# facebookresearch/PointContrast

Hardware: AMD Instinct MI355X
Metric: scene-pairs/sec, ScanNet 2.5cm Res16UNet34C PointInfoNCE (higher is better)
Workload: dtype f32; 1 GPU; BASELINE configs[1]: Res16UNet34C, nce loss, voxel 0.025 m, 4 pairs/GPU, 87380+87371 active voxels per forward pair on rank 0, npos 4096, T 0.4, SGD(lr 0.1, mom 0.8, wd 1e-4); global_batch=4, parallelism=dp1, engine=native, pair_execution=one two-segment pass (BatchNorm statistics per cloud)

## Files before the change

pointcontrast_amd/csrc/spconv_plan.h:

```cpp
#pragma once
#include <algorithm>
#include <cmath>
#include <cstdlib>

#include "internal.h"
#include "spconv_args.h"

namespace pcmi {

constexpr int kStreamKDefaultMinTiles = 256;

struct ConvEnv {
  int64_t sk_min_tiles, conv16_min_rows, conv32r_min_rows;
  bool x3_on;
};
static ConvEnv conv_env() {
  ConvEnv env;
  const char* e = getenv("PCMI_SPCONV_STREAMK");
  env.sk_min_tiles = e ? (int64_t)atoll(e) : (int64_t)kStreamKDefaultMinTiles;
  e = getenv("PCMI_CONV16");
  env.conv16_min_rows = e ? atoll(e) : 512;
  e = getenv("PCMI_CONV16_X3");
  env.x3_on = !e || atoi(e) != 0;
  e = getenv("PCMI_CONV32R");
  env.conv32r_min_rows = e ? (int64_t)atoll(e) : (int64_t)8192;
  return env;
}

static int sk_workgroups_max() { return 4 * num_cu() / 8 * 8; }
static bool sk_rows_eligible(const ConvEnv& env, int64_t rows, int K) {
  const int64_t mt = env.sk_min_tiles;
  return K > 1 && mt > 0 && rows >= 4096  && ceil_div(rows, 128) >= mt;
}
static size_t sk_partial_bytes(const ConvEnv& env, int64_t rows, int N, int K) {
  return sk_rows_eligible(env, rows, K) ? (size_t)sk_workgroups_max() * 2 * 128 * N * sizeof(float) : 0;
}

static bool conv16_enabled(const ConvEnv& env, int64_t n_rows, int64_t x_bytes) {
  const int64_t min_rows = env.conv16_min_rows;
  return min_rows > 0 && n_rows >= min_rows && x_bytes <= 0x7FFFFF00ll;
}

static bool conv16_x3(const ConvEnv& env, int NT, int C, int N) { return env.x3_on && NT >= 2 && NT <= 4 && C >= 64 && N >= 64; }

struct ConvPlan {
  int kernel;
  int RW, NT, ksplit;
  size_t split_bytes, sk_bytes, pack_offset, pack_bytes;
  size_t ws_bytes;
};
constexpr int kMaxKSplit = 27;

static ConvPlan plan_conv(const ConvEnv& env, int64_t rows, int64_t x_bytes, int C, int N, int K, int form) {
  ConvPlan p = {};
  const bool pair = form == PCMI_CONV_FORM_PAIRS, table = form == PCMI_CONV_FORM_TABLE || form == PCMI_CONV_FORM_TABLE_UNITS;
  p.ksplit = 1;
  if (conv32r_eligible(env.conv32r_min_rows, rows, x_bytes, C, N, K, table)) {
    p.kernel = PCMI_CONV_KERNEL_32R;
    return p;
  }
  const bool wide = C >= 64;
  const int nt_all = N / 32;
  p.NT = nt_all % 4 == 0 ? 4 : (nt_all % 3 == 0 ? 3 : (nt_all % 2 == 0 ? 2 : 1));
  p.RW = rows >= 96 ? 4 : (rows >= 48 ? 2 : 1);
  if (p.RW == 1 && p.NT > 2) p.NT = (nt_all % 2 == 0) ? 2 : 1;
  const int64_t min16 = env.conv16_min_rows;
  if (rows < 2048)
    p.NT = (wide && !pair && K > 1 && N >= 64 && nt_all % 2 == 0 && env.x3_on && min16 > 0 && rows >= min16 && p.RW == 4) ? 2 : 1;
  else if (rows < 8192 && p.NT > 2)
    p.NT = (nt_all % 2 == 0) ? 2 : 1;
  if (pair) {
    p.kernel = PCMI_CONV_KERNEL_PAIR;
    return p;
  }
  if (K > 1 && rows > 0) {
    const int64_t wgs = ceil_div(rows, 32 * p.RW) * (nt_all / p.NT);
    const int64_t target = (25 * (int64_t)num_cu()) / 10;
    if (wgs < target) p.ksplit = (int)std::min<int64_t>(std::min<int64_t>(K, kMaxKSplit), ceil_div(target, wgs));
    if (wide && p.RW == 4 && wgs < target && rows < 16384 && conv16_x3(env, p.NT, C, N) && min16 > 0 && rows >= min16) {
      const double slots = (double)x3_workgroups(p.NT, 3), nch = (double)(C / 32);
      const double traffic = (double)rows * N * 8.0 / 3.0e6 / 2.0;
      auto cost = [&](int ks) {
        const double w = (double)wgs * ks;
        const double rounds = std::ceil(w / slots);
        const double thin = std::max(1.0, 2.0 * num_cu() / std::min(w, slots));
        return rounds * ((double)ceil_div((int64_t)K, (int64_t)ks) * nch + 3.0) * thin + traffic * ks;
      };
      int best = p.ksplit;
      const int kmax = (int)std::min<int64_t>(K, kMaxKSplit);
      for (int ks = 1; ks <= kmax; ++ks)
        if (cost(ks) < cost(best) - 1e-9) best = ks;
      if (cost(best) < 0.9 * cost(p.ksplit)) p.ksplit = best;
    }
  }
  const bool c16 = p.RW == 4 && conv16_enabled(env, rows, x_bytes), x3 = conv16_x3(env, p.NT, C, N);
  if (form == PCMI_CONV_FORM_TABLE_UNITS && c16 && p.ksplit == 1 && sk_rows_eligible(env, rows, K) && C >= 64 && N >= 64) {
    p.kernel = x3 ? PCMI_CONV_KERNEL_UNITS_X3 : PCMI_CONV_KERNEL_UNITS_16;
    p.sk_bytes = sk_partial_bytes(env, rows, N, K);
    p.pack_offset = p.sk_bytes;
    p.pack_bytes = x3 ? x3_pack_bytes(K, C, N) : 0;
    p.ws_bytes = p.pack_offset + p.pack_bytes;
    return p;
  }
  p.split_bytes = p.ksplit > 1 ? (size_t)p.ksplit * rows * N * sizeof(float) : 0;
  p.ws_bytes = p.split_bytes;
  if (c16 && x3 && form != PCMI_CONV_FORM_NONE) {
    p.kernel = PCMI_CONV_KERNEL_TABLE_X3;
    p.pack_offset = align_up(p.split_bytes, 256);
    p.pack_bytes = x3_pack_bytes(K, C, N);
    p.ws_bytes = p.pack_offset + p.pack_bytes;
  } else if (c16) {
    p.kernel = PCMI_CONV_KERNEL_TABLE_16;
  } else if (p.RW == 4 && p.NT <= 2 && C % 64 == 0) {
    p.kernel = PCMI_CONV_KERNEL_DEEP;
  } else {
    p.kernel = PCMI_CONV_KERNEL_PLAIN;
  }
  return p;
}

}
```

pointcontrast_amd/csrc/spconv_x3.hip:

```cpp
#include <algorithm>
#include <cstdio>
#include <cstdlib>

#include "common.h"
#include "internal.h"
#include "spconv_args.h"
#include "x3_split.h"

namespace pcmi {

__host__ __device__ constexpr int x3_piece(int n, int kk) { return (n >> 4) * 64 + kk * 16 + (n & 15); }

__host__ __device__ constexpr int x3_channel(int kk, int e) { return 4 * kk + (e & 3) + 16 * (e >> 2); }

template <int TERMS>
__global__ __launch_bounds__(256) void x3_pack_kernel(const float* __restrict__ w, int64_t w_kstride, int64_t w_sc, int64_t w_sn,
                                                      int K, int C, int N, int NS, u32x4* __restrict__ out) {
  const int nch = C / kKC, nns = N / NS;
  const int64_t total = (int64_t)K * nch * nns * NS * 4;
  const int64_t idx = (int64_t)blockIdx.x * 256 + threadIdx.x;
  if (idx >= total) return;
  const int kk = (int)(idx & 3);
  int64_t r = idx >> 2;
  const int nl = (int)(r % NS);
  r /= NS;
  const int ns = (int)(r % nns);
  r /= nns;
  const int cc = (int)(r % nch);
  const int wk = (int)(r / nch);
  const float* wb = w + (int64_t)wk * w_kstride + (int64_t)(ns * NS + nl) * w_sn;
  v4f x0, x1;
#pragma unroll
  for (int e = 0; e < 4; ++e) {
    x0[e] = wb[(int64_t)(cc * kKC + x3_channel(kk, e)) * w_sc];
    x1[e] = wb[(int64_t)(cc * kKC + x3_channel(kk, e + 4)) * w_sc];
  }
  u32x4 h, m, l;
  split_terms<TERMS>(x0, x1, h, m, l);
  u32x4* blk = out + (((int64_t)wk * nch + cc) * nns + ns) * (TERMS * NS * 4);
  const int piece = x3_piece(nl, kk);
  blk[0 * NS * 4 + piece] = h;
  if constexpr (TERMS == 3) {
    blk[1 * NS * 4 + piece] = m;
    blk[2 * NS * 4 + piece] = l;
  }
}

__global__ __launch_bounds__(256) void x3_pack_many_kernel(const X3PackJob* __restrict__ jobs, int n_jobs, int64_t total,
                                                           int64_t item0) {
  const int64_t idx = item0 + (int64_t)blockIdx.x * 256 + threadIdx.x;
  if (idx >= total) return;
  int lo = 0, hi = n_jobs - 1;
  while (lo < hi) {
    const int mid = (lo + hi + 1) >> 1;
    if (jobs[mid].first_item <= idx) lo = mid; else hi = mid - 1;
  }
  const X3PackJob jb = jobs[lo];
  const int64_t loc = idx - jb.first_item;
  const int nch = jb.C / kKC, nns = jb.N / jb.NS;
  const int kk = (int)(loc & 3);
  int64_t r = loc >> 2;
  const int nl = (int)(r % jb.NS);
  r /= jb.NS;
  const int ns = (int)(r % nns);
  r /= nns;
  const int cc = (int)(r % nch);
  const int wk = (int)(r / nch);
  const float* wb = jb.w + (int64_t)wk * jb.w_kstride + (int64_t)(ns * jb.NS + nl) * jb.w_sn;
  v4f x0, x1;
#pragma unroll
  for (int e = 0; e < 4; ++e) {
    x0[e] = wb[(int64_t)(cc * kKC + x3_channel(kk, e)) * jb.w_sc];
    x1[e] = wb[(int64_t)(cc * kKC + x3_channel(kk, e + 4)) * jb.w_sc];
  }
  const int piece = x3_piece(nl, kk);
  if (jb.terms == 1) {
    u32x4 h;
    split1(x0, x1, h);
    reinterpret_cast<u32x4*>(jb.out)[(((int64_t)wk * nch + cc) * nns + ns) * (jb.NS * 4) + piece] = h;
    return;
  }
  u32x4 h, m, l;
  split3(x0, x1, h, m, l);
  u32x4* blk = reinterpret_cast<u32x4*>(jb.out) + (((int64_t)wk * nch + cc) * nns + ns) * (3 * jb.NS * 4);
  blk[0 * jb.NS * 4 + piece] = h;
  blk[1 * jb.NS * 4 + piece] = m;
  blk[2 * jb.NS * 4 + piece] = l;
}

template <int TERMS>
constexpr int x3_min_waves(int NT) { return TERMS == 3 ? (NT == 4 ? 2 : 3) : (NT == 2 ? 4 : 3); }
template <int NT, bool SK, bool DMA, int TERMS>
__global__ __launch_bounds__(256, x3_min_waves<TERMS>(NT)) void spconv16x_kernel(ConvArgs a) {
  constexpr int TM = 128, NS = 32 * NT, CTN = 2 * NT;
  constexpr int KSLOTS = PCMI_MAX_KERNEL_VOLUME;
  constexpr uint32_t kAbsent = 0x80000000u;
  constexpr int kRsrcFlags = 0x00020000;
  constexpr int PIECES = TERMS * NS * 4;
  constexpr int BLOCK_BYTES = PIECES * 16;
  constexpr int BR = (PIECES + 255) / 256;
  static_assert(CTN >= 3, "the three load stages sit behind the MFMAs of column tiles 0, 1, 2");
  __shared__ __attribute__((aligned(16))) u32x4 s_b[2][PIECES];
  __shared__ uint32_t s_off[KSLOTS][TM];
  __shared__ int32_t s_orow[TM];
  __shared__ int2 s_kmeta[KSLOTS];
  __shared__ int32_t s_kabs[KSLOTS];
  __shared__ int32_t s_nk;
  __shared__ int64_t s_tile[2];

  const int n0 = blockIdx.y * NS;
  const int nch = a.C / kKC;
  const uint32_t chunk_bytes = (uint32_t)gridDim.y * BLOCK_BYTES;
  const uint32_t wk_bytes = (uint32_t)nch * chunk_bytes;
  const uint32_t slice_bytes = (uint32_t)blockIdx.y * BLOCK_BYTES;
  int sk_g = 0, sk_tile = 0, sk_u = 0, sk_u1 = 0;
  bool sk_first = true;
  if constexpr (SK) {
    const int G = (int)gridDim.x;
    sk_g = (int)(blockIdx.x & 7) * (G / 8) + (int)(blockIdx.x >> 3);
    const int U = a.sk_pref[a.sk_tiles] * nch;
    const int per = (U + G - 1) / G;
    sk_u = sk_g * per;
    sk_u1 = min(U, sk_u + per);
    if (sk_u >= sk_u1) return;
    if (threadIdx.x < 64) {
      int lo = 0, n = a.sk_tiles;
      while (n > 1) {
        const int stride = (n + 63) / 64;
        const int probe = lo + (int)threadIdx.x * stride;
        const bool le = probe < lo + n && a.sk_pref[probe] * nch <= sk_u;
        const int cnt = __popcll(__ballot(le));
        const int nlo = lo + max(cnt - 1, 0) * stride;
        n = min(stride, lo + n - nlo);
        lo = nlo;
      }
      if (threadIdx.x == 0) s_tile[0] = lo;
    }
    __syncthreads();
    sk_tile = __builtin_amdgcn_readfirstlane((int)s_tile[0]);
  }
  const __amdgpu_buffer_rsrc_t xr = __builtin_amdgcn_make_buffer_rsrc(const_cast<float*>(a.x), 0, 0x7FFFFFFF, kRsrcFlags);
  const __amdgpu_buffer_rsrc_t wr = __builtin_amdgcn_make_buffer_rsrc(const_cast<void*>(a.wpack), 0, 0x7FFFFFFF, kRsrcFlags);
  const uint32_t ld_bytes = (uint32_t)(a.x_ld * 4);
  const int sk_total = SK ? sk_u1 - sk_u : 0;
  int sk_done = 0, prio_qtr = -1;
  for (;;) {
  bool sk_whole = true;
  int sk_next_u = 0, sk_c0 = 0, sk_steps = 0;
  int t = threadIdx.x;
  if constexpr (SK) asm volatile("" : "+v"(t));
  const int lane = t & 63, wave = t >> 6;
  const int i = lane & 15, kk = lane >> 4;
  if constexpr (SK) {
    const int64_t row0 = (int64_t)sk_tile * TM;
    const uint32_t tmask = a.sk_mask[sk_tile];
    const int pref = a.sk_pref[sk_tile] * nch, ns_t = __popc(tmask) * nch;
    const int jb = sk_u - pref, je = min(sk_u1 - pref, ns_t);
    sk_whole = (jb == 0 && je == ns_t);
    sk_next_u = pref + je;
    const int o0 = jb / nch, o1 = (je - 1) / nch;
    sk_c0 = jb - o0 * nch;
    sk_steps = je - jb;
    if (t < a.K && ((tmask >> t) & 1u)) {
      const int j = __popc(tmask & ((1u << t) - 1u));
      if (j >= o0 && j <= o1) {
        s_kabs[j - o0] = t;
        s_kmeta[j - o0] = make_int2(j - o0, (int)((uint32_t)a.wsel[t] * wk_bytes + slice_bytes));
      }
    }
    if (t == 0) s_nk = sk_steps > 0 ? o1 - o0 + 1 : 0;
    if (t < TM) s_orow[t] = (row0 + t < a.n_rows) ? (a.perm ? a.perm[row0 + t] : (int32_t)(row0 + t)) : -1;
    __syncthreads();
    const int cnt = sk_steps > 0 ? o1 - o0 + 1 : 0;
    {
      const int rr = t & (TM - 1);
      const int64_t row = row0 + rr;
      const bool row_ok = row < a.n_rows;
      const int64_t row_c = row_ok ? row : a.n_rows - 1;
      for (int q0 = t >> 7; q0 < cnt; q0 += 8) {
        int32_t v[4];
#pragma unroll
        for (int u = 0; u < 4; ++u) v[u] = a.nbr[(int64_t)s_kabs[min(q0 + 2 * u, cnt - 1)] * a.n_rows + row_c];
#pragma unroll
        for (int u = 0; u < 4; ++u)
          if (q0 + 2 * u < cnt) s_off[q0 + 2 * u][rr] = (row_ok && v[u] >= 0) ? (uint32_t)v[u] * ld_bytes : kAbsent;
      }
    }
  } else {
    int64_t tile = blockIdx.x;
    if (a.xcd_tiles > 0) {
      tile = (int64_t)(blockIdx.x & 7) * a.xcd_tiles + (blockIdx.x >> 3);
      if (tile * TM >= a.n_rows) return;
    }
    const int64_t row0 = tile * TM;
    const int kbeg = (int)((int64_t)a.K * blockIdx.z / a.ksplit);
    const int kend = (int)((int64_t)a.K * (blockIdx.z + 1) / a.ksplit);
    if (t < TM) s_orow[t] = (row0 + t < a.n_rows) ? (a.perm ? a.perm[row0 + t] : (int32_t)(row0 + t)) : -1;
    for (int p = t; p < (kend - kbeg) * TM; p += 256) {
      const int q = p / TM, rr = p - q * TM;
      const int64_t row = row0 + rr;
      int32_t v = -1;
      if (row < a.n_rows) v = a.nbr ? a.nbr[(int64_t)(kbeg + q) * a.n_rows + row] : (int32_t)row;
      s_off[q][rr] = v >= 0 ? (uint32_t)v * ld_bytes : kAbsent;
    }
    __syncthreads();
    if (t < 64) {
      int nk = 0;
      for (int q = 0; q < kend - kbeg; ++q) {
        bool any = false;
        for (int rr = t; rr < TM; rr += 64) any |= (s_off[q][rr] != kAbsent);
        if (__any(any)) {
          if (t == 0) s_kmeta[nk] = make_int2(q, (int)((uint32_t)a.wsel[kbeg + q] * wk_bytes + slice_bytes));
          ++nk;
        }
      }
      if (t == 0) s_nk = nk;
    }
  }
  __syncthreads();
  const int nk = s_nk;
  const int nsteps = SK ? sk_steps : nk * nch;

  f32x4 acc[2][CTN];
#pragma unroll
  for (int g = 0; g < 2; ++g)
#pragma unroll
    for (int ct = 0; ct < CTN; ++ct) acc[g][ct] = (f32x4){0.f, 0.f, 0.f, 0.f};

  constexpr int BRR = DMA ? 1 : BR;
  uint32_t bvo[BRR];
#pragma unroll
  for (int q = 0; q < BRR; ++q) bvo[q] = (t + q * 256 < PIECES) ? (uint32_t)(t + q * 256) * 16u : kAbsent;
  u32x4 breg[BRR];
  auto store_b = [&](int buf) {
    if constexpr (!DMA) {
#pragma unroll
      for (int q = 0; q < BR; ++q)
        if ((q + 1) * 256 <= PIECES || t + q * 256 < PIECES) s_b[buf][t + q * 256] = breg[q];
    }
  };
  constexpr int WPIECES = PIECES / 64, WR = (WPIECES + 3) / 4;
  const int wave_u = __builtin_amdgcn_readfirstlane(wave);
  auto dma_b = [&](int buf, uint32_t soff) {
    if constexpr (DMA) {
#pragma unroll
      for (int r = 0; r < WR; ++r) {
        const int wp = wave_u + 4 * r;
        if (wp < WPIECES)
          __builtin_amdgcn_raw_ptr_buffer_load_lds(wr, (__attribute__((address_space(3))) void*)&s_b[buf][wp * 64], 16,
                                                   (uint32_t)lane * 16u,
                                                   (uint32_t)__builtin_amdgcn_readfirstlane((int)(soff + (uint32_t)wp * 1024u)), 0, 0);
      }
    }
  };
  v4f a0[2][2], a1[2][2];
  int va0 = 0, va1 = 0;
  int lj = 0, lc = sk_c0 - 1;
  int2 l_meta = make_int2(0, 0);
  uint32_t l_voff[2] = {kAbsent, kAbsent};
  const uint32_t off_lane = (uint32_t)(wave * 32 + i) * 4;
  auto stage_meta = [&]() {
    ++lc;
    if (lc == nch) {
      lc = 0;
      ++lj;
    }
    lc = __builtin_amdgcn_readfirstlane(lc);
    lj = __builtin_amdgcn_readfirstlane(lj);
    l_meta = s_kmeta[min(lj, KSLOTS - 1)];
  };
  auto stage_b = [&](bool live, int nbuf) {
    const int krow = __builtin_amdgcn_readfirstlane(l_meta.x) & 31;
    const uint32_t wofs = (uint32_t)__builtin_amdgcn_readfirstlane(l_meta.y);
    const char* row = reinterpret_cast<const char*>(&s_off[0][0]) + min(krow, KSLOTS - 1) * (TM * 4) + off_lane;
    l_voff[0] = *reinterpret_cast<const uint32_t*>(row);
    l_voff[1] = *reinterpret_cast<const uint32_t*>(row + 64);
    const uint32_t soff = (uint32_t)__builtin_amdgcn_readfirstlane((int)(wofs + (uint32_t)lc * chunk_bytes));
    if constexpr (DMA) {
      if (live) dma_b(nbuf, soff);
    } else {
#pragma unroll
      for (int q = 0; q < BR; ++q)
        breg[q] = __builtin_bit_cast(u32x4, __builtin_amdgcn_raw_buffer_load_b128(wr, live ? bvo[q] : kAbsent, live ? soff : 0u, 0));
    }
  };
  auto stage_a = [&](v4f (&dst)[2][2], bool live) -> int {
    const uint32_t v0 = live ? l_voff[0] : kAbsent, v1 = live ? l_voff[1] : kAbsent;
    const int va = (__any(v0 != kAbsent) ? 1 : 0) | (__any(v1 != kAbsent) ? 2 : 0);
    const uint32_t soff = (uint32_t)__builtin_amdgcn_readfirstlane(lc * (kKC * 4));
    const uint32_t o0 = v0 + 16 * kk, o1 = v1 + 16 * kk;
    dst[0][0] = __builtin_bit_cast(v4f, __builtin_amdgcn_raw_buffer_load_b128(xr, o0, soff, 0));
    dst[1][0] = __builtin_bit_cast(v4f, __builtin_amdgcn_raw_buffer_load_b128(xr, o1, soff, 0));
    dst[0][1] = __builtin_bit_cast(v4f, __builtin_amdgcn_raw_buffer_load_b128(xr, o0 + 64, soff, 0));
    dst[1][1] = __builtin_bit_cast(v4f, __builtin_amdgcn_raw_buffer_load_b128(xr, o1 + 64, soff, 0));
    return va;
  };

  if (nsteps > 0) {
    stage_meta();
    stage_b(true, 0);
    va0 = stage_a(a0, true);
    store_b(0);
    __syncthreads();
    auto do_step = [&](int step, v4f (&cur)[2][2], int va_cur, v4f (&nxt)[2][2], int& va_nxt) {
      const bool more = step + 1 < nsteps;
      if constexpr (SK) {
        const int qtr = __builtin_amdgcn_readfirstlane(((sk_done + step) * 4) / max(sk_total, 1));
        if (qtr != prio_qtr) {
          prio_qtr = qtr;
          if (qtr <= 0) __builtin_amdgcn_s_setprio(3);
          else if (qtr == 1) __builtin_amdgcn_s_setprio(2);
          else if (qtr == 2) __builtin_amdgcn_s_setprio(1);
          else __builtin_amdgcn_s_setprio(0);
        }
      }
      const bool g0 = (va_cur & 1) != 0, g1 = (va_cur & 2) != 0;
      u32x4 ah[2], am[2], al[2];
      if (g0) split_terms<TERMS>(cur[0][0], cur[0][1], ah[0], am[0], al[0]);
      if (g1) split_terms<TERMS>(cur[1][0], cur[1][1], ah[1], am[1], al[1]);
      const u32x4* sb = &s_b[step & 1][kk * 16 + i];
      u32x4 bh[2], bm[2], bl[2];
      if (va_cur) {
        bh[0] = sb[0 * NS * 4];
        if constexpr (TERMS == 3) {
          bm[0] = sb[1 * NS * 4];
          bl[0] = sb[2 * NS * 4];
        }
      }
      __builtin_amdgcn_sched_barrier(0);
#pragma unroll
      for (int ct = 0; ct < CTN; ++ct) {
        const int rb = ct & 1;
        if (va_cur && ct + 1 < CTN) {
          bh[rb ^ 1] = sb[(0 * NS + 16 * (ct + 1)) * 4];
          if constexpr (TERMS == 3) {
            bm[rb ^ 1] = sb[(1 * NS + 16 * (ct + 1)) * 4];
            bl[rb ^ 1] = sb[(2 * NS + 16 * (ct + 1)) * 4];
          }
        }
#define PCMI_X3_MFMA(G, AT, BT)                                                                                             \
  acc[G][ct] = __builtin_amdgcn_mfma_f32_16x16x32_bf16(__builtin_bit_cast(bf16x8, AT[G]), __builtin_bit_cast(bf16x8, BT[rb]), \
                                                       acc[G][ct], 0, 0, 0)
#define PCMI_X3_SIX(G)        \
  if constexpr (TERMS == 3) { \
    PCMI_X3_MFMA(G, al, bh);  \
    PCMI_X3_MFMA(G, ah, bl);  \
    PCMI_X3_MFMA(G, am, bm);  \
    PCMI_X3_MFMA(G, am, bh);  \
    PCMI_X3_MFMA(G, ah, bm);  \
  }                           \
  PCMI_X3_MFMA(G, ah, bh)
        if (g0 && g1) {
          PCMI_X3_SIX(0);
          PCMI_X3_SIX(1);
        } else if (g0) {
          PCMI_X3_SIX(0);
        } else if (g1) {
          PCMI_X3_SIX(1);
        }
#undef PCMI_X3_SIX
#undef PCMI_X3_MFMA
        if (ct == 0) stage_meta();
        if (ct == 1) stage_b(more, (step + 1) & 1);
        if (ct == 2) va_nxt = stage_a(nxt, more);
        __builtin_amdgcn_sched_barrier(0);
      }
      if (more) store_b((step + 1) & 1);
      __syncthreads();
    };
    for (int step = 0; step < nsteps; step += 2) {
      do_step(step, a0, va0, a1, va1);
      if (step + 1 < nsteps) do_step(step + 1, a1, va1, a0, va0);
    }
  }

  if (SK && !sk_whole) {
    float* pp = a.sk_part + ((int64_t)(2 * sk_g + (sk_first ? 0 : 1)) * TM + wave * 32) * a.N + n0 + i;
#pragma unroll
    for (int g = 0; g < 2; ++g)
#pragma unroll
      for (int r = 0; r < 4; ++r) {
        const int rl = g * 16 + 4 * kk + r;
#pragma unroll
        for (int ct = 0; ct < CTN; ++ct) pp[(int64_t)rl * a.N + ct * 16] = acc[g][ct][r];
      }
  } else {
    float* outp = a.out + (int64_t)blockIdx.z * a.split_stride;
    float bv[CTN];
#pragma unroll
    for (int ct = 0; ct < CTN; ++ct) bv[ct] = a.bias ? a.bias[n0 + ct * 16 + i] : 0.f;
#pragma unroll
    for (int g = 0; g < 2; ++g)
#pragma unroll
      for (int r = 0; r < 4; ++r) {
        const int32_t orow = s_orow[wave * 32 + g * 16 + 4 * kk + r];
        if (orow >= 0) {
          float* op = outp + (int64_t)orow * a.out_ld + n0 + i;
          if (a.accumulate) {
#pragma unroll
            for (int ct = 0; ct < CTN; ++ct) op[ct * 16] += acc[g][ct][r] + bv[ct];
          } else {
#pragma unroll
            for (int ct = 0; ct < CTN; ++ct) op[ct * 16] = acc[g][ct][r] + bv[ct];
          }
        }
      }
  }
  if constexpr (!SK) {
    break;
  } else {
    sk_u = sk_next_u;
    ++sk_tile;
    sk_first = false;
    sk_done += nsteps;
    if (sk_u >= sk_u1) break;
    __syncthreads();
  }
  }
}

template <bool SK, bool DMA, int TERMS>
static int launch_x3(int NT, const ConvArgs& a, dim3 grid, hipStream_t st) {
  switch (NT) {
    case 2: spconv16x_kernel<2, SK, DMA, TERMS><<<grid, 256, 0, st>>>(a); break;
    case 3: spconv16x_kernel<3, SK, DMA, TERMS><<<grid, 256, 0, st>>>(a); break;
    case 4: spconv16x_kernel<4, SK, DMA, TERMS><<<grid, 256, 0, st>>>(a); break;
    default: set_error("spconv x3: bad NT %d", NT); return PCMI_ERR_INVALID;
  }
  PCMI_LAUNCH_CHECK();
  return PCMI_OK;
}

size_t x3_pack_bytes(int K, int C, int N) { return align_up((size_t)std::max(K, 1) * C * N * 6, 256); }

int x3_workgroups(int NT, int terms) {
  return (terms == 1 ? x3_min_waves<1>(NT) : x3_min_waves<3>(NT)) * num_cu() / 8 * 8;
}

int x3_pack_weights(const ConvArgs& a, int NT, void* out, hipStream_t st, int terms) {
  PCMI_REQUIRE(out && ((uintptr_t)out % 16 == 0) && a.C % kKC == 0 && a.N % (32 * NT) == 0 && (terms == 1 || terms == 3),
               PCMI_ERR_INVALID, "spconv x3: bad pack arguments (%d -> %d, NT %d, %d terms)", a.C, a.N, NT, terms);
  const int64_t total = (int64_t)a.K * (a.C / kKC) * a.N * 4;
  const dim3 grid((unsigned)ceil_div(total, 256));
  if (terms == 1)
    x3_pack_kernel<1><<<grid, 256, 0, st>>>(a.w, a.w_kstride, a.w_sc, a.w_sn, a.K, a.C, a.N, 32 * NT, reinterpret_cast<u32x4*>(out));
  else
    x3_pack_kernel<3><<<grid, 256, 0, st>>>(a.w, a.w_kstride, a.w_sc, a.w_sn, a.K, a.C, a.N, 32 * NT, reinterpret_cast<u32x4*>(out));
  PCMI_LAUNCH_CHECK();
  return PCMI_OK;
}

int x3_pack_many(const X3PackJob* jobs_dev, int n_jobs, int64_t total_items, hipStream_t st, int64_t first_item) {
  if (n_jobs <= 0 || total_items <= first_item) return PCMI_OK;
  x3_pack_many_kernel<<<dim3((unsigned)ceil_div(total_items - first_item, 256)), 256, 0, st>>>(jobs_dev, n_jobs, total_items, first_item);
  PCMI_LAUNCH_CHECK();
  return PCMI_OK;
}

static thread_local const X3Prepacked* t_prepacked = nullptr;
static thread_local int t_n_prepacked = 0;
void x3_set_prepacked(const X3Prepacked* table, int n) {
  t_prepacked = table;
  t_n_prepacked = table ? n : 0;
}
const void* x3_find_prepacked(const float* w, bool transposed, int NT, int terms) {
  for (int i = 0; i < t_n_prepacked; ++i)
    if (t_prepacked[i].w == w && (t_prepacked[i].transposed != 0) == transposed && t_prepacked[i].NT == NT &&
        t_prepacked[i].terms == terms)
      return t_prepacked[i].pack;
  return nullptr;
}

int x3_launch(int NT, bool sk, const ConvArgs& a, dim3 grid, hipStream_t st, int terms) {
  PCMI_REQUIRE(a.wpack && NT >= 2 && NT <= 4 && (terms == 1 || terms == 3), PCMI_ERR_INVALID,
               "spconv x3: needs packed weights, NT in 2..4 and 1 or 3 terms (NT %d, %d terms)", NT, terms);
  if (terms == 1) return sk ? launch_x3<true, true, 1>(NT, a, grid, st) : launch_x3<false, true, 1>(NT, a, grid, st);
  return sk ? launch_x3<true, true, 3>(NT, a, grid, st) : launch_x3<false, true, 3>(NT, a, grid, st);
}

}
```

Measured before the change: 294.1 scene-pairs/sec.

## Run NT=4 three-term x3 conv with eight one-group waves per workgroup

Adds a template parameter so each wave can own one 16-row group instead of two. For the three-term NT=4 path, the default launch becomes 512 threads with eight waves, cutting the per-wave accumulator and A-register footprint. The aim is more latency hiding and fewer register limits at the same tile size. This costs more waves sharing the same LDS B tile, smaller per-wave MFMA batches and a different occupancy hint; an environment variable restores the four-wave layout.

```diff
diff --git a/pointcontrast_amd/csrc/spconv_plan.h b/pointcontrast_amd/csrc/spconv_plan.h
--- a/pointcontrast_amd/csrc/spconv_plan.h
+++ b/pointcontrast_amd/csrc/spconv_plan.h
@@ -12,7 +12,7 @@
 
 struct ConvEnv {
   int64_t sk_min_tiles, conv16_min_rows, conv32r_min_rows;
-  bool x3_on;
+  bool x3_on, x3_four_waves;
 };
 static ConvEnv conv_env() {
   ConvEnv env;
@@ -22,6 +22,8 @@
   env.conv16_min_rows = e ? atoll(e) : 512;
   e = getenv("PCMI_CONV16_X3");
   env.x3_on = !e || atoi(e) != 0;
+  e = getenv("PCMI_CONV16X_WAVES");
+  env.x3_four_waves = e && atoi(e) == 4;
   e = getenv("PCMI_CONV32R");
   env.conv32r_min_rows = e ? (int64_t)atoll(e) : (int64_t)8192;
   return env;
diff --git a/pointcontrast_amd/csrc/spconv_x3.hip b/pointcontrast_amd/csrc/spconv_x3.hip
--- a/pointcontrast_amd/csrc/spconv_x3.hip
+++ b/pointcontrast_amd/csrc/spconv_x3.hip
@@ -5,6 +5,7 @@
 #include "common.h"
 #include "internal.h"
 #include "spconv_args.h"
+#include "spconv_plan.h"
 #include "x3_split.h"
 
 namespace pcmi {
@@ -90,15 +91,19 @@
 
 template <int TERMS>
 constexpr int x3_min_waves(int NT) { return TERMS == 3 ? (NT == 4 ? 2 : 3) : (NT == 2 ? 4 : 3); }
-template <int NT, bool SK, bool DMA, int TERMS>
-__global__ __launch_bounds__(256, x3_min_waves<TERMS>(NT)) void spconv16x_kernel(ConvArgs a) {
+template <int TERMS>
+constexpr bool x3_one_group(int NT) { return TERMS == 3 && NT == 4; }
+template <int NT, bool SK, bool DMA, int TERMS, int GW>
+__global__ __launch_bounds__(512 / GW, x3_min_waves<TERMS>(NT) * 2 / GW) void spconv16x_kernel(ConvArgs a) {
   constexpr int TM = 128, NS = 32 * NT, CTN = 2 * NT;
+  constexpr int WAVES = 8 / GW, THREADS = 64 * WAVES;
+  static_assert(GW == 1 || GW == 2, "a wave holds one or two 16-row groups");
   constexpr int KSLOTS = PCMI_MAX_KERNEL_VOLUME;
   constexpr uint32_t kAbsent = 0x80000000u;
   constexpr int kRsrcFlags = 0x00020000;
   constexpr int PIECES = TERMS * NS * 4;
   constexpr int BLOCK_BYTES = PIECES * 16;
-  constexpr int BR = (PIECES + 255) / 256;
+  constexpr int BR = (PIECES + THREADS - 1) / THREADS;
   static_assert(CTN >= 3, "the three load stages sit behind the MFMAs of column tiles 0, 1, 2");
   __shared__ __attribute__((aligned(16))) u32x4 s_b[2][PIECES];
   __shared__ uint32_t s_off[KSLOTS][TM];
@@ -173,17 +178,18 @@
     __syncthreads();
     const int cnt = sk_steps > 0 ? o1 - o0 + 1 : 0;
     {
+      constexpr int QS = THREADS / TM;
       const int rr = t & (TM - 1);
       const int64_t row = row0 + rr;
       const bool row_ok = row < a.n_rows;
       const int64_t row_c = row_ok ? row : a.n_rows - 1;
-      for (int q0 = t >> 7; q0 < cnt; q0 += 8) {
+      for (int q0 = t >> 7; q0 < cnt; q0 += 4 * QS) {
         int32_t v[4];
 #pragma unroll
-        for (int u = 0; u < 4; ++u) v[u] = a.nbr[(int64_t)s_kabs[min(q0 + 2 * u, cnt - 1)] * a.n_rows + row_c];
+        for (int u = 0; u < 4; ++u) v[u] = a.nbr[(int64_t)s_kabs[min(q0 + QS * u, cnt - 1)] * a.n_rows + row_c];
 #pragma unroll
         for (int u = 0; u < 4; ++u)
-          if (q0 + 2 * u < cnt) s_off[q0 + 2 * u][rr] = (row_ok && v[u] >= 0) ? (uint32_t)v[u] * ld_bytes : kAbsent;
+          if (q0 + QS * u < cnt) s_off[q0 + QS * u][rr] = (row_ok && v[u] >= 0) ? (uint32_t)v[u] * ld_bytes : kAbsent;
       }
     }
   } else {
@@ -196,7 +202,7 @@
     const int kbeg = (int)((int64_t)a.K * blockIdx.z / a.ksplit);
     const int kend = (int)((int64_t)a.K * (blockIdx.z + 1) / a.ksplit);
     if (t < TM) s_orow[t] = (row0 + t < a.n_rows) ? (a.perm ? a.perm[row0 + t] : (int32_t)(row0 + t)) : -1;
-    for (int p = t; p < (kend - kbeg) * TM; p += 256) {
+    for (int p = t; p < (kend - kbeg) * TM; p += THREADS) {
       const int q = p / TM, rr = p - q * TM;
       const int64_t row = row0 + rr;
       int32_t v = -1;
@@ -221,31 +227,31 @@
   const int nk = s_nk;
   const int nsteps = SK ? sk_steps : nk * nch;
 
-  f32x4 acc[2][CTN];
-#pragma unroll
-  for (int g = 0; g < 2; ++g)
+  f32x4 acc[GW][CTN];
+#pragma unroll
+  for (int g = 0; g < GW; ++g)
 #pragma unroll
     for (int ct = 0; ct < CTN; ++ct) acc[g][ct] = (f32x4){0.f, 0.f, 0.f, 0.f};
 
   constexpr int BRR = DMA ? 1 : BR;
   uint32_t bvo[BRR];
 #pragma unroll
-  for (int q = 0; q < BRR; ++q) bvo[q] = (t + q * 256 < PIECES) ? (uint32_t)(t + q * 256) * 16u : kAbsent;
+  for (int q = 0; q < BRR; ++q) bvo[q] = (t + q * THREADS < PIECES) ? (uint32_t)(t + q * THREADS) * 16u : kAbsent;
   u32x4 breg[BRR];
   auto store_b = [&](int buf) {
     if constexpr (!DMA) {
 #pragma unroll
       for (int q = 0; q < BR; ++q)
-        if ((q + 1) * 256 <= PIECES || t + q * 256 < PIECES) s_b[buf][t + q * 256] = breg[q];
+        if ((q + 1) * THREADS <= PIECES || t + q * THREADS < PIECES) s_b[buf][t + q * THREADS] = breg[q];
     }
   };
-  constexpr int WPIECES = PIECES / 64, WR = (WPIECES + 3) / 4;
+  constexpr int WPIECES = PIECES / 64, WR = (WPIECES + WAVES - 1) / WAVES;
   const int wave_u = __builtin_amdgcn_readfirstlane(wave);
   auto dma_b = [&](int buf, uint32_t soff) {
     if constexpr (DMA) {
 #pragma unroll
       for (int r = 0; r < WR; ++r) {
-        const int wp = wave_u + 4 * r;
+        const int wp = wave_u + WAVES * r;
         if (wp < WPIECES)
           __builtin_amdgcn_raw_ptr_buffer_load_lds(wr, (__attribute__((address_space(3))) void*)&s_b[buf][wp * 64], 16,
                                                    (uint32_t)lane * 16u,
@@ -253,12 +259,14 @@
       }
     }
   };
-  v4f a0[2][2], a1[2][2];
+  v4f a0[GW][2], a1[GW][2];
   int va0 = 0, va1 = 0;
   int lj = 0, lc = sk_c0 - 1;
   int2 l_meta = make_int2(0, 0);
-  uint32_t l_voff[2] = {kAbsent, kAbsent};
-  const uint32_t off_lane = (uint32_t)(wave * 32 + i) * 4;
+  uint32_t l_voff[GW];
+#pragma unroll
+  for (int g = 0; g < GW; ++g) l_voff[g] = kAbsent;
+  const uint32_t off_lane = (uint32_t)(wave * (16 * GW) + i) * 4;
   auto stage_meta = [&]() {
     ++lc;
     if (lc == nch) {
@@ -273,8 +281,8 @@
     const int krow = __builtin_amdgcn_readfirstlane(l_meta.x) & 31;
     const uint32_t wofs = (uint32_t)__builtin_amdgcn_readfirstlane(l_meta.y);
     const char* row = reinterpret_cast<const char*>(&s_off[0][0]) + min(krow, KSLOTS - 1) * (TM * 4) + off_lane;
-    l_voff[0] = *reinterpret_cast<const uint32_t*>(row);
-    l_voff[1] = *reinterpret_cast<const uint32_t*>(row + 64);
+#pragma unroll
+    for (int g = 0; g < GW; ++g) l_voff[g] = *reinterpret_cast<const uint32_t*>(row + 64 * g);
     const uint32_t soff = (uint32_t)__builtin_amdgcn_readfirstlane((int)(wofs + (uint32_t)lc * chunk_bytes));
     if constexpr (DMA) {
       if (live) dma_b(nbuf, soff);
@@ -284,15 +292,21 @@
         breg[q] = __builtin_bit_cast(u32x4, __builtin_amdgcn_raw_buffer_load_b128(wr, live ? bvo[q] : kAbsent, live ? soff : 0u, 0));
     }
   };
-  auto stage_a = [&](v4f (&dst)[2][2], bool live) -> int {
-    const uint32_t v0 = live ? l_voff[0] : kAbsent, v1 = live ? l_voff[1] : kAbsent;
-    const int va = (__any(v0 != kAbsent) ? 1 : 0) | (__any(v1 != kAbsent) ? 2 : 0);
+  auto stage_a = [&](v4f (&dst)[GW][2], bool live) -> int {
+    uint32_t o[GW];
+    int va = 0;
+#pragma unroll
+    for (int g = 0; g < GW; ++g) {
+      const uint32_t v = live ? l_voff[g] : kAbsent;
+      va |= __any(v != kAbsent) ? (1 << g) : 0;
+      o[g] = v + 16 * kk;
+    }
     const uint32_t soff = (uint32_t)__builtin_amdgcn_readfirstlane(lc * (kKC * 4));
-    const uint32_t o0 = v0 + 16 * kk, o1 = v1 + 16 * kk;
-    dst[0][0] = __builtin_bit_cast(v4f, __builtin_amdgcn_raw_buffer_load_b128(xr, o0, soff, 0));
-    dst[1][0] = __builtin_bit_cast(v4f, __builtin_amdgcn_raw_buffer_load_b128(xr, o1, soff, 0));
-    dst[0][1] = __builtin_bit_cast(v4f, __builtin_amdgcn_raw_buffer_load_b128(xr, o0 + 64, soff, 0));
-    dst[1][1] = __builtin_bit_cast(v4f, __builtin_amdgcn_raw_buffer_load_b128(xr, o1 + 64, soff, 0));
+#pragma unroll
+    for (int h = 0; h < 2; ++h)
+#pragma unroll
+      for (int g = 0; g < GW; ++g)
+        dst[g][h] = __builtin_bit_cast(v4f, __builtin_amdgcn_raw_buffer_load_b128(xr, o[g] + 64 * h, soff, 0));
     return va;
   };
 
@@ -302,7 +316,7 @@
     va0 = stage_a(a0, true);
     store_b(0);
     __syncthreads();
-    auto do_step = [&](int step, v4f (&cur)[2][2], int va_cur, v4f (&nxt)[2][2], int& va_nxt) {
+    auto do_step = [&](int step, v4f (&cur)[GW][2], int va_cur, v4f (&nxt)[GW][2], int& va_nxt) {
       const bool more = step + 1 < nsteps;
       if constexpr (SK) {
         const int qtr = __builtin_amdgcn_readfirstlane(((sk_done + step) * 4) / max(sk_total, 1));
@@ -314,10 +328,11 @@
           else __builtin_amdgcn_s_setprio(0);
         }
       }
-      const bool g0 = (va_cur & 1) != 0, g1 = (va_cur & 2) != 0;
-      u32x4 ah[2], am[2], al[2];
+      const bool g0 = (va_cur & 1) != 0, g1 = GW == 2 && (va_cur & 2) != 0;
+      u32x4 ah[GW], am[GW], al[GW];
       if (g0) split_terms<TERMS>(cur[0][0], cur[0][1], ah[0], am[0], al[0]);
-      if (g1) split_terms<TERMS>(cur[1][0], cur[1][1], ah[1], am[1], al[1]);
+      if constexpr (GW == 2)
+        if (g1) split_terms<TERMS>(cur[1][0], cur[1][1], ah[1], am[1], al[1]);
       const u32x4* sb = &s_b[step & 1][kk * 16 + i];
       u32x4 bh[2], bm[2], bl[2];
       if (va_cur) {
@@ -350,13 +365,17 @@
     PCMI_X3_MFMA(G, ah, bm);  \
   }                           \
   PCMI_X3_MFMA(G, ah, bh)
-        if (g0 && g1) {
-          PCMI_X3_SIX(0);
-          PCMI_X3_SIX(1);
+        if constexpr (GW == 2) {
+          if (g0 && g1) {
+            PCMI_X3_SIX(0);
+            PCMI_X3_SIX(1);
+          } else if (g0) {
+            PCMI_X3_SIX(0);
+          } else if (g1) {
+            PCMI_X3_SIX(1);
+          }
         } else if (g0) {
           PCMI_X3_SIX(0);
-        } else if (g1) {
-          PCMI_X3_SIX(1);
         }
 #undef PCMI_X3_SIX
 #undef PCMI_X3_MFMA
@@ -375,9 +394,9 @@
   }
 
   if (SK && !sk_whole) {
-    float* pp = a.sk_part + ((int64_t)(2 * sk_g + (sk_first ? 0 : 1)) * TM + wave * 32) * a.N + n0 + i;
-#pragma unroll
-    for (int g = 0; g < 2; ++g)
+    float* pp = a.sk_part + ((int64_t)(2 * sk_g + (sk_first ? 0 : 1)) * TM + wave * (16 * GW)) * a.N + n0 + i;
+#pragma unroll
+    for (int g = 0; g < GW; ++g)
 #pragma unroll
       for (int r = 0; r < 4; ++r) {
         const int rl = g * 16 + 4 * kk + r;
@@ -390,10 +409,10 @@
 #pragma unroll
     for (int ct = 0; ct < CTN; ++ct) bv[ct] = a.bias ? a.bias[n0 + ct * 16 + i] : 0.f;
 #pragma unroll
-    for (int g = 0; g < 2; ++g)
+    for (int g = 0; g < GW; ++g)
 #pragma unroll
       for (int r = 0; r < 4; ++r) {
-        const int32_t orow = s_orow[wave * 32 + g * 16 + 4 * kk + r];
+        const int32_t orow = s_orow[wave * (16 * GW) + g * 16 + 4 * kk + r];
         if (orow >= 0) {
           float* op = outp + (int64_t)orow * a.out_ld + n0 + i;
           if (a.accumulate) {
@@ -420,11 +439,19 @@
 }
 
 template <bool SK, bool DMA, int TERMS>
-static int launch_x3(int NT, const ConvArgs& a, dim3 grid, hipStream_t st) {
+static int launch_x3(int NT, bool four_waves, const ConvArgs& a, dim3 grid, hipStream_t st) {
   switch (NT) {
-    case 2: spconv16x_kernel<2, SK, DMA, TERMS><<<grid, 256, 0, st>>>(a); break;
-    case 3: spconv16x_kernel<3, SK, DMA, TERMS><<<grid, 256, 0, st>>>(a); break;
-    case 4: spconv16x_kernel<4, SK, DMA, TERMS><<<grid, 256, 0, st>>>(a); break;
+    case 2: spconv16x_kernel<2, SK, DMA, TERMS, 2><<<grid, 256, 0, st>>>(a); break;
+    case 3: spconv16x_kernel<3, SK, DMA, TERMS, 2><<<grid, 256, 0, st>>>(a); break;
+    case 4:
+      if constexpr (x3_one_group<TERMS>(4)) {
+        if (!four_waves) {
+          spconv16x_kernel<4, SK, DMA, TERMS, 1><<<grid, 512, 0, st>>>(a);
+          break;
+        }
+      }
+      spconv16x_kernel<4, SK, DMA, TERMS, 2><<<grid, 256, 0, st>>>(a);
+      break;
     default: set_error("spconv x3: bad NT %d", NT); return PCMI_ERR_INVALID;
   }
   PCMI_LAUNCH_CHECK();
@@ -474,8 +501,9 @@
 int x3_launch(int NT, bool sk, const ConvArgs& a, dim3 grid, hipStream_t st, int terms) {
   PCMI_REQUIRE(a.wpack && NT >= 2 && NT <= 4 && (terms == 1 || terms == 3), PCMI_ERR_INVALID,
                "spconv x3: needs packed weights, NT in 2..4 and 1 or 3 terms (NT %d, %d terms)", NT, terms);
-  if (terms == 1) return sk ? launch_x3<true, true, 1>(NT, a, grid, st) : launch_x3<false, true, 1>(NT, a, grid, st);
-  return sk ? launch_x3<true, true, 3>(NT, a, grid, st) : launch_x3<false, true, 3>(NT, a, grid, st);
-}
-
-}
+  const bool w4 = conv_env().x3_four_waves;
+  if (terms == 1) return sk ? launch_x3<true, true, 1>(NT, w4, a, grid, st) : launch_x3<false, true, 1>(NT, w4, a, grid, st);
+  return sk ? launch_x3<true, true, 3>(NT, w4, a, grid, st) : launch_x3<false, true, 3>(NT, w4, a, grid, st);
+}
+
+}
```

Result: no change. 293.9 scene-pairs/sec (median of 2 runs) (-0.1%).
